# BayesWatch/deep-kernel-transfer

Hardware: AMD Instinct MI355X
Metric: episodes/sec (higher is better)
Workload: dtype f32/f16x2-split

## Files before the change

deep-kernel-transfer_amd/csrc/dkt_mll.h:

```cpp
#pragma once
#include "dkt_common.h"
#include "../../include/dkt_abi.h"

struct MllArgs {
    const float* E;
    const float* Y;
    long y_bstride;
    const float* sv;
    const float* mean;
    const float* noise;
    const float* cls_weight;
    float* logp;
    float* alpha;
    float* L;
    float* W;
    float* dsv;
    float* dmean;
    float* dnoise;
    float* jitter_used;
    int32_t* info;
    float* ws;
    const int32_t* only_failed;
    int b0;
    int B, C, N, LD;
    float jitter0;
    int max_tries;
    unsigned flags;
    int p2_guard;
    float kappa_max = 0.f;
};

constexpr float DKT_HALF_LOG_2PI = 0.91893853320467274178f;

bool dkt_mll_h2_launch(const MllArgs& a, hipStream_t st);
bool dkt_mll_mfma_launch(const MllArgs& a, hipStream_t st);
bool dkt_mll_reg_launch(const MllArgs& a, hipStream_t st);

void dkt_chol_inv_block_launch(const float* A, int lda, long sA, float* L, int ldl, long sL, float* U, int ldu, long sU, int nb,
                               int pivot_base, int32_t* info, int nmat, hipStream_t st);
size_t dkt_mll_big_workspace_bytes(int B, int C, int N);
int dkt_mll_big_launch(const MllArgs& a, void* workspace, size_t ws_bytes, hipStream_t st);
bool dkt_mll_tiled_supports(int N, unsigned flags, int C = 1);
size_t dkt_mll_tiled_workspace_bytes(int B, int C, int N);
size_t dkt_mll_tiled_workspace_bytes_form(int B, int C, int N, bool per_class);
int dkt_mll_tiled_launch(const MllArgs& a, void* workspace, size_t ws_bytes, hipStream_t st);
bool dkt_mll_band_supports(int N, unsigned flags, int C);
bool dkt_mll_band_applies(int B, int C, int N, unsigned flags);
size_t dkt_mll_band_workspace_bytes(int B, int C, int N);
int dkt_mll_band_launch(const MllArgs& a, void* workspace, size_t ws_bytes, hipStream_t st);
void dkt_mll_generic_global_launch(MllArgs a, int b0, int count, float* ws, hipStream_t st);
size_t dkt_mll_generic_global_floats(int count, int N);
```

deep-kernel-transfer_amd/csrc/dkt_mll.hip:

```cpp
#include "dkt_mll.h"
#include <cstdlib>

namespace {

constexpr size_t MLL_LDS_LIMIT = 150 * 1024;

__host__ __device__ inline int mll_ld(int N) { return N | 1; }
inline size_t mll_vec_floats(int N) { return (size_t)3 * (N + 1) + 32; }
inline size_t mll_mat_floats(int N) { return (size_t)(N + 1) * mll_ld(N); }
inline bool mll_fits_lds(int N) { return (mll_vec_floats(N) + mll_mat_floats(N)) * 4 <= MLL_LDS_LIMIT; }

template <bool GLOBAL>
__global__ __launch_bounds__(256) void mll_generic_kernel(MllArgs a) {
    extern __shared__ __attribute__((aligned(16))) float smem[];
    const int tid = threadIdx.x;
    const int tx = tid & 15, ty = tid >> 4;
    const int N = a.N, C = a.C, LD = a.LD, R = N + 1;
    const bool epc = (a.flags & DKT_MLL_E_PER_CLASS) != 0;
    const size_t unit = epc ? (size_t)a.b0 * C + blockIdx.x : (size_t)a.b0 + blockIdx.x;
    const int b = epc ? (int)(unit / (size_t)C) : (int)unit;
    const int c_first = epc ? (int)(unit % (size_t)C) : 0, c_end = epc ? c_first + 1 : C;
    if (a.only_failed) {
        bool need = false;
        for (int c = c_first; c < c_end; ++c) need = need || a.only_failed[(size_t)b * C + c] != 0;
        if (!need) return;
        __syncthreads();
    }
    float* cs = smem;
    float* ldiag = cs + R;
    float* al = ldiag + R;
    float* red = al + R;
    float* Mw = GLOBAL ? (a.ws + (size_t)blockIdx.x * R * LD) : (red + 32);
#define MW(p, j) Mw[(p) * LD + (j)]

    const float* Eb = a.E + unit * N * N;
    const bool want_grad = (a.flags & DKT_MLL_WANT_GRAD) != 0;
    const bool want_chol = (a.flags & DKT_MLL_WANT_CHOL) != 0;
    float* Wb = want_grad ? a.W + unit * N * N : nullptr;

    for (int c = c_first; c < c_end; ++c) {
        const float svc = a.sv[c], mc = a.mean[c], nzc = a.noise[c];
        const float* yc = a.Y + (size_t)b * a.y_bstride + (size_t)c * N;
        int fail_at = 0;
        float jit = 0.f;
        for (int attempt = 0; attempt <= a.max_tries; ++attempt) {
            jit = 0.f;
            if (attempt > 0) {
                jit = a.jitter0;
                for (int i = 1; i < attempt; ++i) jit *= 10.f;
            }
            __syncthreads();
            for (int idx = tid; idx < N * N; idx += 256) {
                const int p = idx / N, j = idx - p * N;
                float v = 0.f;
                if (p >= j) {
                    v = svc * Eb[idx];
                    if (p == j) v += nzc + jit;
                }
                MW(p, j) = v;
            }
            for (int j = tid; j < N; j += 256) MW(N, j) = yc[j] - mc;
            __syncthreads();
            fail_at = 0;
            for (int k = 0; k < N; ++k) {
                const float d = MW(k, k);
                if (!(d > 0.f)) { fail_at = k + 1; break; }
                const float lkk = sqrtf(d);
                const float rinv = 1.0f / lkk;
                for (int p = tid; p < R; p += 256) {
                    if (p != k) {
                        const float v = MW(p, k) * rinv;
                        cs[p] = v;
                        MW(p, k) = v;
                    } else {
                        cs[p] = rinv;
                        ldiag[k] = lkk;
                    }
                }
                __syncthreads();
                for (int p = ty; p < R; p += 16) {
                    const bool low = p <= k;
                    const float cp = cs[p];
                    for (int j = k + 1 + tx; j < N; j += 16) {
                        if (low || p >= j) MW(p, j) -= cp * cs[j];
                    }
                }
                __syncthreads();
            }
            if (fail_at == 0) break;
        }
        __syncthreads();
        const size_t bc = (size_t)b * C + c;
        if (fail_at != 0) {
            const float qnan = __int_as_float(0x7fc00000);
            if (tid == 0) {
                a.logp[bc] = qnan;
                a.jitter_used[bc] = jit;
                a.info[bc] = fail_at;
                if (want_grad) { a.dsv[bc] = qnan; a.dmean[bc] = qnan; a.dnoise[bc] = qnan; }
            }
            for (int i = tid; i < N; i += 256) a.alpha[bc * N + i] = qnan;
            if (want_grad)
                for (int idx = tid; idx < N * N; idx += 256) Wb[idx] = qnan;
            if (want_chol)
                for (int idx = tid; idx < N * N; idx += 256) a.L[bc * N * N + idx] = qnan;
            continue;
        }
        for (int k = tid; k < N; k += 256) MW(k, k) = 1.0f / ldiag[k];
        __syncthreads();
        float qpart = 0.f, lpart = 0.f;
        for (int k = tid; k < N; k += 256) {
            const float w = MW(N, k);
            qpart += w * w;
            lpart += logf(ldiag[k]);
        }
        const float quad = block_sum_256(qpart, red);
        const float logdet_half = block_sum_256(lpart, red);
        float apart = 0.f;
        for (int i = tid; i < N; i += 256) {
            float s = 0.f;
            for (int m = i; m < N; ++m) s += MW(i, m) * MW(N, m);
            al[i] = s;
            a.alpha[bc * N + i] = s;
            apart += s;
        }
        const float asum = block_sum_256(apart, red);
        if (tid == 0) {
            a.logp[bc] = -0.5f * quad - logdet_half - (float)N * DKT_HALF_LOG_2PI;
            a.jitter_used[bc] = jit;
            a.info[bc] = 0;
        }
        if (want_chol) {
            float* Lb = a.L + bc * N * N;
            for (int idx = tid; idx < N * N; idx += 256) {
                const int p = idx / N, j = idx - p * N;
                Lb[idx] = (p > j) ? MW(p, j) : (p == j ? ldiag[p] : 0.f);
            }
        }
        if (want_grad) {
            const float cw = a.cls_weight ? a.cls_weight[c] : 1.0f;
            const float coef = cw * svc;
            float dsv_part = 0.f, tr_part = 0.f;
            for (int i = ty; i < N; i += 16) {
                for (int j = tx; j <= i; j += 16) {
                    float kinv = 0.f;
                    for (int m = i; m < N; ++m) kinv += MW(i, m) * MW(j, m);
                    const float mcv = 0.5f * (al[i] * al[j] - kinv);
                    const float e = Eb[(size_t)i * N + j];
                    if (i == j) { dsv_part += mcv * e; tr_part += mcv; }
                    else dsv_part += 2.0f * mcv * e;
                    const float wv = coef * mcv;
                    if (c == c_first) {
                        Wb[(size_t)i * N + j] = wv;
                        if (i != j) Wb[(size_t)j * N + i] = wv;
                    } else {
                        Wb[(size_t)i * N + j] += wv;
                        if (i != j) Wb[(size_t)j * N + i] += wv;
                    }
                }
            }
            const float dsv = block_sum_256(dsv_part, red);
            const float trm = block_sum_256(tr_part, red);
            if (tid == 0) {
                a.dsv[bc] = dsv;
                a.dmean[bc] = asum;
                a.dnoise[bc] = trm;
            }
        }
    }
#undef MW
}

}

size_t dkt_mll_generic_global_floats(int count, int N) { return (size_t)count * mll_mat_floats(N); }

void dkt_mll_generic_global_launch(MllArgs a, int b0, int count, float* ws, hipStream_t st) {
    a.b0 = b0; a.ws = ws; a.LD = mll_ld(a.N);
    const int units = (a.flags & DKT_MLL_E_PER_CLASS) ? count * a.C : count;
    hipLaunchKernelGGL(mll_generic_kernel<true>, dim3(units), dim3(256), mll_vec_floats(a.N) * sizeof(float), st, a);
}

constexpr float MLL_H2_KAPPA_MAX = 5.0e3f;

static bool mll_kappa_guarded(const MllArgs& a) { return !(a.flags & DKT_MLL_NO_KAPPA_GUARD) && mll_fits_lds(a.N); }

static void mll_kappa_fixup(MllArgs a, hipStream_t st) {
    if (!mll_kappa_guarded(a)) return;
    const int upe = (a.flags & DKT_MLL_E_PER_CLASS) ? a.C : 1;
    const size_t units = (size_t)a.B * upe;
    a.only_failed = a.info;
    a.b0 = 0; a.LD = mll_ld(a.N);
    const size_t lds = (mll_vec_floats(a.N) + mll_mat_floats(a.N)) * sizeof(float);
    if (lds > 48 * 1024 && hipFuncSetAttribute((const void*)mll_generic_kernel<false>, hipFuncAttributeMaxDynamicSharedMemorySize, (int)lds) != hipSuccess) return;
    hipLaunchKernelGGL(mll_generic_kernel<false>, dim3((unsigned)units), dim3(256), lds, st, a);
}

static int g_mll_env_read = 0, g_p2_guard = 1, g_force_f32mfma = 0;
void dkt_mll_reload_env() { g_mll_env_read = 0; }

extern "C" size_t dkt_mll_workspace_bytes(int B, int C, int N) {
    if (B <= 0 || N <= 0 || C <= 0) return 0;
    if (N + 1 <= 128) return 0;
    const size_t big = dkt_mll_big_workspace_bytes(B, C, N);
    const size_t gen = mll_fits_lds(N) ? 0 : (size_t)B * mll_mat_floats(N) * sizeof(float);
    const size_t til = dkt_mll_tiled_supports(N, 0) ? dkt_mll_tiled_workspace_bytes(B, C, N) : 0;
    const size_t bnd = dkt_mll_band_supports(N, 0, C) ? dkt_mll_band_workspace_bytes(B, C, N) : 0;
    size_t mx = big > gen ? big : gen;
    mx = mx > bnd ? mx : bnd;
    return mx > til ? mx : til;
}

extern "C" size_t dkt_mll_workspace_bytes_for(int B, int C, int N, unsigned flags) {
    if (B <= 0 || N <= 0 || C <= 0) return 0;
    const bool pc = (flags & DKT_MLL_E_PER_CLASS) != 0;
    const size_t gen = mll_fits_lds(N) ? 0 : (size_t)(pc ? (B < 128 ? B : 128) * C : B) * mll_mat_floats(N) * sizeof(float);
    if (flags & DKT_MLL_FORCE_GENERIC) return gen;
    if (N + 1 <= 128) return (flags & DKT_MLL_WANT_CHOL) && (N + 1 + 15) / 16 > 2 ? gen : 0;
    if (dkt_mll_band_applies(B, C, N, flags)) return dkt_mll_band_workspace_bytes(B, C, N);
    if (!(flags & DKT_MLL_FORCE_BLOCKED) && dkt_mll_tiled_supports(N, flags, C)) return dkt_mll_tiled_workspace_bytes_form(B, C, N, pc);
    if (pc) return gen;
    const size_t big = dkt_mll_big_workspace_bytes(B, C, N);
    return big > gen ? big : gen;
}

extern "C" int dkt_mll_f32(const float* E, const float* Y, long y_bstride, const float* sv, const float* mean,
                           const float* noise, int B, int C, int N, float jitter0, int max_tries,
                           unsigned flags, const float* cls_weight, float* logp, float* alpha, float* L,
                           float* W, float* dsv, float* dmean, float* dnoise, float* jitter_used,
                           int32_t* info, void* workspace, size_t workspace_bytes, void* stream) {
    if (!E || !Y || !sv || !mean || !noise || !logp || !alpha || !jitter_used || !info) return DKT_ERR_BAD_ARG;
    if (B <= 0 || C <= 0 || N <= 0 || max_tries < 0 || max_tries > 8 || y_bstride < 0) return DKT_ERR_BAD_ARG;
    if ((flags & DKT_MLL_WANT_GRAD) && (!W || !dsv || !dmean || !dnoise)) return DKT_ERR_BAD_ARG;
    if ((flags & DKT_MLL_WANT_CHOL) && !L) return DKT_ERR_BAD_ARG;
    MllArgs a;
    a.E = E; a.Y = Y; a.y_bstride = y_bstride; a.sv = sv; a.mean = mean; a.noise = noise;
    a.cls_weight = cls_weight; a.logp = logp; a.alpha = alpha; a.L = L; a.W = W; a.dsv = dsv;
    a.dmean = dmean; a.dnoise = dnoise; a.jitter_used = jitter_used; a.info = info;
    a.ws = (float*)workspace; a.only_failed = nullptr; a.b0 = 0; a.B = B; a.C = C; a.N = N; a.LD = mll_ld(N);
    a.jitter0 = jitter0; a.max_tries = max_tries; a.flags = flags;
    if (g_mll_env_read == 0) {
        const char* pg = dkt_variant_env("DKT_MLL_P2_GUARD");
        g_p2_guard = pg ? atoi(pg) : 1;
        const char* fm = getenv("DKT_MLL_F32MFMA");
        g_force_f32mfma = (fm && fm[0] == '1') ? 1 : 0;
        g_mll_env_read = 1;
    }
    a.p2_guard = g_p2_guard;
    if (g_force_f32mfma && !(flags & (DKT_MLL_E_PER_CLASS | DKT_MLL_FORCE_GENERIC | DKT_MLL_FORCE_REG | DKT_MLL_FORCE_BLOCKED))) {
        flags |= DKT_MLL_FORCE_F32MFMA;
        a.flags = flags;
    }
    hipStream_t st = (hipStream_t)stream;
    if (flags & DKT_MLL_FORCE_REG) return DKT_ERR_BAD_ARG;
    if (flags & DKT_MLL_E_PER_CLASS) {
        if (flags & (DKT_MLL_WANT_CHOL | DKT_MLL_FORCE_REG | DKT_MLL_FORCE_F32MFMA | DKT_MLL_FORCE_BLOCKED)) return DKT_ERR_BAD_ARG;
        if (!(flags & DKT_MLL_FORCE_GENERIC)) {
            if (N + 1 > 128 && dkt_mll_tiled_supports(N, flags, C)) {
                if (!workspace || workspace_bytes < dkt_mll_tiled_workspace_bytes_form(B, C, N, true)) return DKT_ERR_WORKSPACE;
                return dkt_mll_tiled_launch(a, workspace, workspace_bytes, st);
            }
            if (N + 1 <= 128) {
                a.kappa_max = mll_kappa_guarded(a) ? MLL_H2_KAPPA_MAX : 0.f;
                if (!dkt_mll_h2_launch(a, st)) return DKT_ERR_BAD_ARG;
                mll_kappa_fixup(a, st);
                return hipGetLastError() == hipSuccess ? DKT_OK : DKT_ERR_LAUNCH;
            }
        }
    }
    a.kappa_max = (N + 1 <= 128 && mll_kappa_guarded(a)) ? MLL_H2_KAPPA_MAX : 0.f;
    if (!(flags & (DKT_MLL_FORCE_GENERIC | DKT_MLL_FORCE_REG | DKT_MLL_FORCE_F32MFMA)) && dkt_mll_h2_launch(a, st)) {
        mll_kappa_fixup(a, st);
        return hipGetLastError() == hipSuccess ? DKT_OK : DKT_ERR_LAUNCH;
    }
    if (!(flags & (DKT_MLL_FORCE_GENERIC | DKT_MLL_FORCE_REG)) && dkt_mll_mfma_launch(a, st)) return hipGetLastError() == hipSuccess ? DKT_OK : DKT_ERR_LAUNCH;
    if (dkt_mll_band_applies(B, C, N, flags) && workspace && workspace_bytes >= dkt_mll_band_workspace_bytes(B, C, N))
        return dkt_mll_band_launch(a, workspace, workspace_bytes, st);
    if (!(flags & (DKT_MLL_FORCE_GENERIC | DKT_MLL_FORCE_REG | DKT_MLL_FORCE_BLOCKED)) && dkt_mll_tiled_supports(N, flags, C) && workspace &&
        workspace_bytes >= dkt_mll_tiled_workspace_bytes_form(B, C, N, false))
        return dkt_mll_tiled_launch(a, workspace, workspace_bytes, st);
    if (!(flags & (DKT_MLL_FORCE_GENERIC | DKT_MLL_E_PER_CLASS)) && N + 1 > 128 && workspace && workspace_bytes >= dkt_mll_big_workspace_bytes(B, C, N))
        return dkt_mll_big_launch(a, workspace, workspace_bytes, st);
    const int upe = (flags & DKT_MLL_E_PER_CLASS) ? C : 1;
    if (mll_fits_lds(N)) {
        const size_t lds = (mll_vec_floats(N) + mll_mat_floats(N)) * sizeof(float);
        if (lds > 48 * 1024) {
            if (hipFuncSetAttribute((const void*)mll_generic_kernel<false>,
                                    hipFuncAttributeMaxDynamicSharedMemorySize, (int)lds) != hipSuccess)
                return DKT_ERR_LAUNCH;
        }
        hipLaunchKernelGGL(mll_generic_kernel<false>, dim3((unsigned)B * upe), dim3(256), lds, st, a);
    } else {
        const size_t per_ep = (size_t)upe * mll_mat_floats(N) * sizeof(float);
        const size_t fit = workspace ? workspace_bytes / per_ep : 0;
        if (fit < 1) return DKT_ERR_WORKSPACE;
        const int cnt = fit < (size_t)B ? (int)fit : B;
        for (int b0 = 0; b0 < B; b0 += cnt) dkt_mll_generic_global_launch(a, b0, (B - b0 < cnt) ? B - b0 : cnt, (float*)workspace, st);
    }
    return hipGetLastError() == hipSuccess ? DKT_OK : DKT_ERR_LAUNCH;
}
```

deep-kernel-transfer_amd/csrc/dkt_mll_h2.hip:

```cpp
#include "dkt_h2_tiles.h"
#include <cstdlib>

namespace {

using namespace dkt_mfma;

#ifndef DKT_H2E_P2H
#define DKT_H2E_P2H 1
#endif
#ifndef DKT_H2_SWEEP_PRIO
#define DKT_H2_SWEEP_PRIO 1
#endif
#define DKT_SWEEP_PRIO(p) do { if (DKT_H2_SWEEP_PRIO) __builtin_amdgcn_s_setprio(p); } while (0)

constexpr int ntt(int nt) { return nt * (nt + 1) / 2; }
__host__ __device__ constexpr int tidx(int i, int j) { return j * (j + 1) / 2 + i; }

constexpr int H2_MAX_WPG = 5;

#ifdef DKT_MFMA_CLOCKS
#define DKT_CLK(i) do { __builtin_amdgcn_sched_barrier(0); clk[i] = __builtin_amdgcn_s_memtime(); __builtin_amdgcn_sched_barrier(0); } while (0)
#else
#define DKT_CLK(i) do { } while (0)
#endif
// ... 398 lines not shown
            float asum = 0.f, aa = 0.f;
            {
                const brsrc ar = mk_rsrc(a.alpha + bc * N, (unsigned)(N * 4));
                const float asc = ldexpf(aug_unscale, -msc);
                float* ysf = reinterpret_cast<float*>(myys);
#pragma unroll
                for (int i = 0; i < NT; ++i) {
                    const f32x4 m = (i < NT - 1) ? T.t[i][NT - 1] : myst[(NT - 1) * 64 + lane];
                    const float v = -(qn == 0 ? m[0] : qn == 1 ? m[1] : qn == 2 ? m[2] : m[3]) * asc;
                    const bool ok = arow && ((i < NT - 1) || (c16 < pN));
                    bstore1(ar, (fail_at != 0) ? qnan : v, ok ? (16 * i + c16) * 4 : OOB, 0);
                    if (GRAD && arow) ysf[16 * i + c16] = ok ? v : 0.f;
                    asum += ok ? v : 0.f;
                    aa += ok ? v * v : 0.f;
                }
            }
            float trk = 0.f;
            DKT_CLK(4);
            if constexpr (GRAD) {
                float mx = 0.f;
#pragma unroll
                for (int i = 0; i < NT - 1; ++i) {
#pragma unroll
                    for (int q = 0; q < 4; ++q) T.t[i][NT - 1][q] = (g4 + q == pN) ? 0.f : T.t[i][NT - 1][q];
                }
#pragma unroll
                for (int j = 1; j < NT; ++j) {
#pragma unroll
                    for (int i = 0; i < j; ++i) {
                        const f32x4 v = T.t[i][j];
                        mx = fmaxf(mx, fmaxf(fmaxf(fabsf(v[0]), fabsf(v[1])), fmaxf(fabsf(v[2]), fabsf(v[3]))));
                    }
                }
#pragma unroll
                for (int j = 0; j < NT; ++j) {
                    const f32x4 v = myst[j * 64 + lane];
#pragma unroll
                    for (int q = 0; q < 4; ++q) mx = fmaxf(mx, (j == NT - 1 && g4 + q == pN) ? 0.f : fabsf(v[q]));
                }
                mx = wave_reduce_dpp<true>(mx);
                mx = __int_as_float(__builtin_amdgcn_readfirstlane(__float_as_int(mx)));
                float s3_inv;
                const float s3 = scale_for(mx, s3_inv);
#pragma unroll
                for (int j = 0; j < NT; ++j) {
                    f32x4 v = myst[j * 64 + lane];
                    if (j == NT - 1) {
#pragma unroll
                        for (int q = 0; q < 4; ++q) v[q] = (g4 + q == pN) ? 0.f : v[q];
                    }
                    myst[j * 64 + lane] = split_h2(v, s3);
                }
#pragma unroll
                for (int j = 1; j < NT; ++j) {
#pragma unroll
                    for (int i = 0; i < j; ++i) T.t[i][j] = split_h2(T.t[i][j], s3);
                }
#pragma unroll
                for (int j = 0; j < NT; ++j) {
                    __builtin_amdgcn_sched_barrier(0);
#pragma unroll
                    for (int i = 0; i <= j; i += 2) {
                        const bool pair = i + 1 <= j;
                        f32x4 accA = {0.f, 0.f, 0.f, 0.f}, accB = {0.f, 0.f, 0.f, 0.f};
#pragma unroll
                        for (int k = j; k < NT; ++k) {
                            const f32x4 Bm = (k == j) ? myst[k * 64 + lane] : T.t[j][k];
                            const f32x4 A0 = (k == i) ? myst[k * 64 + lane] : T.t[i][k];
                            if (pair) {
                                const f32x4 A1 = (k == i + 1) ? myst[k * 64 + lane] : T.t[i + 1][k];
                                xtyh2(A0, Bm, accA, A1, Bm, accB);
                            } else {
                                accA = xtyh(A0, Bm, accA);
                            }
                        }
                        auto put = [&](const f32x4 acc, const int ii) {
                            if (ii < j) {
                                T.t[ii][j] = acc;
                            } else {
                                myst[j * 64 + lane] = acc;
#pragma unroll
                                for (int q = 0; q < 4; ++q) {
                                    const bool ok = (g4 + q == c16) && ((j < NT - 1) || (c16 < pN));
                                    trk += ok ? acc[q] : 0.f;
                                }
                            }
                        };
                        put(accA, i);
                        if (pair) put(accB, i + 1);
                    }
                }
                trk *= s3_inv * s3_inv * ldexpf(1.0f, -2 * msc);
                const float cw = a.cls_weight ? a.cls_weight[c] : 1.0f;
                coefK = (fail_at == 0) ? -0.5f * cw * a.sv[c] * s3_inv * s3_inv * ldexpf(1.0f, -2 * msc) : qnan;
                coefA = 0.5f * cw * a.sv[c];
            }
            DKT_CLK(5);
            lsum = wave_reduce_dpp<false>(lsum) + (float)(2 * msc * N);
            asum = wave_reduce_dpp<false>(asum);
            aa = wave_reduce_dpp<false>(aa);
            trk = wave_reduce_dpp<false>(trk);
            if (lane == 0) {
                const bool ok = fail_at == 0;
                a.logp[bc] = ok ? (-0.5f * quad - 0.34657359027997264f * lsum - (float)N * DKT_HALF_LOG_2PI) : qnan;
                a.jitter_used[bc] = jit;
                a.info[bc] = (ok && kappa_high) ? -1 : fail_at;
                if constexpr (GRAD) {
                    const float nz_eff = a.noise[c] + jit;
                    const float trpp = trk - aa;
                    a.dmean[bc] = ok ? asum : qnan;
                    a.dnoise[bc] = ok ? -0.5f * trpp : qnan;
                    a.dsv[bc] = ok ? 0.5f * ((quad - (float)N) + nz_eff * trpp) / a.sv[c] : qnan;
                }
            }
        }
        DKT_CLK(6);
        if constexpr (GRAD) {
            __syncthreads();
            tq = tid;
            DKT_OPAQUE_V(tq);
            c16 = tq & 15; g4 = (tq >> 2) & 12; lane = tq & 63;
            DKT_OPAQUE_S(N);
            const int pNs = N - 16 * (NT - 1);
            const brsrc Wr = mk_rsrc(a.W + (size_t)unit * N * N, (unsigned)(N * N * 4));
            const float* alf = reinterpret_cast<const float*>(myys);
            auto scaled_tile = [&](const f32x4 p, const int i, const int j) {
                const f32x4 ar = myys[4 * i + (g4 >> 2)];
                const float ac = alf[16 * j + c16] * coefA;
                f32x4 v;
#pragma unroll
                for (int q = 0; q < 4; ++q) v[q] = fmaf(ar[q], ac, p[q] * coefK);
                return v;
            };
            auto store_tile = [&](f32x4 v, const int i, const int j) {
                const bool col_ok = (j < NT - 1) || (c16 < pNs);
                const int vo_m = col_ok ? ((16 * j + c16) * N + 16 * i + g4) * 4 : OOB;
                int vo_d[4], vo_t[4];
#pragma unroll
                for (int q = 0; q < 4; ++q) {
                    const bool row_ok = (i < NT - 1) || (g4 + q < pNs);
                    const bool keep = row_ok && col_ok && (i < j || g4 + q <= c16);
                    vo_d[q] = keep ? ((16 * i + g4 + q) * N + 16 * j + c16) * 4 : OOB;
                    vo_t[q] = (keep && g4 + q < c16) ? ((16 * j + c16) * N + 16 * i + g4 + q) * 4 : OOB;
                }
                if (round > 0) {
                    if (i < j) {
                        v += bload4(Wr, vo_m, 0);
                    } else {
#pragma unroll
                        for (int q = 0; q < 4; ++q) v[q] += __uint_as_float(__builtin_amdgcn_raw_buffer_load_b32(Wr, vo_d[q], 0, 0));
                    }
                }
#pragma unroll
                for (int q = 0; q < 4; ++q) bstore1(Wr, v[q], vo_d[q], 0);
                if (i < j) bstore4(Wr, v, vo_m, 0);
                else {
#pragma unroll
                    for (int q = 0; q < 4; ++q) bstore1(Wr, v[q], vo_t[q], 0);
                }
            };
            if constexpr (WPG5) {
                constexpr int KMAX = (NTT + 4) / 5;
#pragma unroll
                for (int g = 0; g < 5; ++g) {
                    if (ep_ok) {
#pragma unroll
                        for (int j = 0; j < NT; ++j) {
#pragma unroll
                            for (int i = 0; i <= j; ++i) {
                                const int n = tidx(i, j);
                                if (n % 5 != g) continue;
                                f32x4 v = {0.f, 0.f, 0.f, 0.f};
                                if (active) v = scaled_tile((i < j) ? T.t[i][j] : myst[j * 64 + lane], i, j);
                                stage[(w * KMAX + n / 5) * 64 + lane] = v;
                            }
                        }
                    }
                    __syncthreads();
                    if (ep_ok) {
                        for (int k = w; 5 * k + g < NTT; k += 5) {
                            f32x4 v = stage[k * 64 + lane];
#pragma unroll
                            for (int ww = 1; ww < 5; ++ww) v += stage[(ww * KMAX + k) * 64 + lane];
                            const int n = 5 * k + g;
                            int j = 0;
                            while ((j + 1) * (j + 2) / 2 <= n) ++j;
                            store_tile(v, n - j * (j + 1) / 2, j);
                        }
                    }
                    if (g < 4 || round + 1 < nrounds) __syncthreads();
                }
            } else {
                for (int t = 0; t < wpg; ++t) {
                    if (t == w && active) {
#pragma unroll
                        for (int j = 0; j < NT; ++j) {
#pragma unroll
                            for (int i = 0; i <= j; ++i) {
                                f32x4 v = scaled_tile((i < j) ? T.t[i][j] : myst[j * 64 + lane], i, j);
                                f32x4* p = &stage[tidx(i, j) * 64 + lane];
                                if (t > 0) v += *p;
                                *p = v;
                            }
                        }
                    }
                    __syncthreads();
                }
                if (ep_ok) {
                    for (int n = w; n < NTT; n += wpg) {
                        int j = 0;
                        while ((j + 1) * (j + 2) / 2 <= n) ++j;
                        store_tile(stage[n * 64 + lane], n - j * (j + 1) / 2, j);
                    }
                }
                if (round + 1 < nrounds) __syncthreads();
            }
        } else {
            if (round + 1 < nrounds) __syncthreads();
        }
    }
    DKT_CLK(7);
#ifdef DKT_MFMA_CLOCKS
    DKT_CLK(8);
    if ((tid & 63) == 0 && a.ws) {
        unsigned long long* o = reinterpret_cast<unsigned long long*>(a.ws) + ((size_t)blockIdx.x * (H2_MAX_WPG * EPW) + wall) * 48;
        for (int i = 0; i < 32; ++i) o[i] = clk[i];
    }
#endif
}

template <int NT> constexpr int h2e_wlds() { return ntt(NT) < 19 ? ntt(NT) : 19; }

template <int NT>
__global__ __attribute__((amdgpu_flat_work_group_size(64, 64), amdgpu_waves_per_eu(2, 2)))
void mll_h2e_kernel(MllArgs a) {
    constexpr int WLDS = h2e_wlds<NT>();
    constexpr int WREG = ntt(NT) - WLDS;
    __shared__ f32x4 wl[WLDS * 64];
    __shared__ f32x4 yst[NT * 4];

    const bool epc = (a.flags & DKT_MLL_E_PER_CLASS) != 0;
    const bool want_grad = (a.flags & DKT_MLL_WANT_GRAD) != 0;
    const int C = a.C;
    const int b = epc ? (int)(blockIdx.x / (unsigned)C) : (int)blockIdx.x;
    const int c_first = epc ? (int)(blockIdx.x % (unsigned)C) : 0, c_end = epc ? c_first + 1 : C;
    const size_t mat = epc ? (size_t)b * C + c_first : (size_t)b;
    const float qnan = __int_as_float(0x7fc00000);
    int tq = threadIdx.x;
    DKT_OPAQUE_V(tq);
    int c16 = tq & 15, g4 = (tq >> 2) & 12, lane = tq & 63, N = a.N;
    DKT_OPAQUE_S(N);

    f32x4 wr[WREG > 0 ? WREG : 1];
#pragma unroll
    for (int n = 0; n < WREG; ++n) wr[n] = (f32x4){0.f, 0.f, 0.f, 0.f};
#pragma unroll
    for (int n = 0; n < WLDS; ++n) wl[n * 64 + lane] = (f32x4){0.f, 0.f, 0.f, 0.f};
#ifdef DKT_MFMA_CLOCKS
    unsigned long long ph[8] = {}, tprev = __builtin_amdgcn_s_memtime();
#define DKT_PH(i) do { __builtin_amdgcn_sched_barrier(0); const unsigned long long tn = __builtin_amdgcn_s_memtime(); ph[i] += tn - tprev; tprev = tn; __builtin_amdgcn_sched_barrier(0); } while (0)
#else
#define DKT_PH(i) do { } while (0)
#endif
    int e_acc = -1000;
    float sigma = 0.f;
    bool poison = false;

    int attempt = 0;
    for (int c = c_first; c < c_end;) {
        tq = threadIdx.x;
        DKT_OPAQUE_V(tq);
        c16 = tq & 15; g4 = (tq >> 2) & 12; lane = tq & 63; N = a.N;
        DKT_OPAQUE_S(N);
        const int pN = N - 16 * (NT - 1);
        Lane ln;
        ln.lane = lane; ln.g = g4 >> 2; ln.c = c16;
        ln.g0 = ln.g == 0; ln.g1 = ln.g == 1; ln.g2 = ln.g == 2;
        const float svc = a.sv[c], mc = a.mean[c], nzc = a.noise[c];
        const size_t bc = (size_t)b * C + c;
        float r2 = 0.f;
        {
            const brsrc yr = mk_rsrc(a.Y + (size_t)b * a.y_bstride + (size_t)c * N, (unsigned)(N * 4));
            float* ysf = reinterpret_cast<float*>(yst);
            {
                const float yv = __uint_as_float(__builtin_amdgcn_raw_buffer_load_b32(yr, lane * 4, 0, 0));
                if (lane < 16 * NT) ysf[lane] = yv;
                r2 = (lane < N) ? (yv - mc) * (yv - mc) : 0.f;
            }
            if (NT > 4 && lane + 64 < 16 * NT) {
                const float yv = __uint_as_float(__builtin_amdgcn_raw_buffer_load_b32(yr, (lane + 64) * 4, 0, 0));
                ysf[lane + 64] = yv;
                r2 += (lane + 64 < N) ? (yv - mc) * (yv - mc) : 0.f;
            }
        }
        r2 = wave_reduce_dpp<false>(r2);
        h4 negIh;
#pragma unroll
        for (int q = 0; q < 4; ++q) negIh[q] = (g4 + q == c16) ? (_Float16)-1.0f : (_Float16)0.0f;
        FormCtxT<true> f;
        f.es = nullptr; f.ys = yst;
        f.pN = pN; f.c16 = c16; f.g4 = g4; f.lane = lane; f.mc = mc;
        Tiles<NT> T;
        int fail_at = 0;
        bool kappa_high = false;
        float jit = 0.f, lsum = 0.f, quad = 0.f, aug_unscale = 1.f;
        int msc = 0;
        const brsrc Er = mk_rsrc(a.E + mat * N * N, (unsigned)(N * N * 4));
        {
            if (attempt > 0) {
                jit = a.jitter0;
                for (int i = 1; i < attempt; ++i) jit *= 10.f;
            }
            load_all_e<NT>(T, Er, N, pN, c16, g4);
            float emax = 0.f, etr = 0.f;
#pragma unroll
            for (int j = 0; j < NT; ++j) {
#pragma unroll
                for (int q = 0; q < 4; ++q) {
                    emax = fmaxf(emax, (g4 + q == c16) ? T.t[j][j][q] : 0.f);
                    etr += (g4 + q == c16) ? T.t[j][j][q] : 0.f;
                }
            }
            emax = wave_reduce_dpp<true>(emax);
            kappa_high = a.kappa_max > 0.f && !(1.0f + svc * wave_reduce_dpp<false>(etr) / nzc <= a.kappa_max);
            int ex;
            (void)frexpf(fmaf(svc, emax, nzc + jit), &ex);
            msc = max(0, (ex + 1) >> 1);
            const float ikap = ldexpf(1.0f, -2 * msc);
            const float lam = fmaxf((nzc + jit) * ikap, 9.094947017729282e-13f);
            int exm;
            (void)frexpf(1.0f / lam, &exm);
            const int emu = (exm + 1) >> 1;
            int exr;
            (void)frexpf(r2 * ikap * ldexpf(1.0f, 2 * emu), &exr);
            const int er = (r2 > 0.f) ? ((exr + 1) >> 1) : 0;
            f.nsv = -svc * ikap * TWO30;
            f.dg = -(nzc + jit) * ikap * TWO30;
            f.rsc = ldexpf(TWO30, -msc - er);
            aug_unscale = ldexpf(1.0f, er);
            form_row0<NT, 0>(T, f);
            DKT_PH(0);
            P1Ctx pc;
            pc.myst = nullptr; pc.negIh = negIh;
            pc.lane = lane; pc.c16 = c16; pc.pN = pN;
            pc.fail_at = 0; pc.lsum = 0.f; pc.quad = 0.f;
#ifdef DKT_MFMA_CLOCKS
            unsigned long long clkdummy[32];
            pc.clk = clkdummy;
#endif
            {
                float dv, x[16];
                sweep_begin30(T.t[0][0], x, dv);
                sweep_interleaved<NT, -1, 0, NT == 1>(T, f, x, dv, ln, pN);
                phase1_step<NT, 0>(T, f, pc, x, dv, ln);
            }
            fail_at = pc.fail_at; lsum = pc.lsum; quad = pc.quad * aug_unscale * aug_unscale;
        }
        DKT_PH(1);
        if (fail_at != 0 && attempt < a.max_tries) {
            ++attempt;
            continue;
        }
        tq = threadIdx.x;
        DKT_OPAQUE_V(tq);
        c16 = tq & 15; g4 = (tq >> 2) & 12; lane = tq & 63;
#if DKT_H2E_P2H
        const float cw = a.cls_weight ? a.cls_weight[c] : 1.0f;
        const float wmag = 0.5f * fabsf(cw) * svc;
        const float gsc = (wmag > 0.f) ? __builtin_sqrtf(wmag) * ldexpf(1.0f, -msc) : ldexpf(1.0f, -msc);
        const bool arow = (ln.g == (pN >> 2));
        const int qn = pN & 3;
        const float asc = ldexpf(aug_unscale, -msc);
        float asum = 0.f, aa = 0.f;
        const brsrc ar = mk_rsrc(a.alpha + bc * N, (unsigned)(N * 4));
        float* ysf = reinterpret_cast<float*>(yst);
        auto emit_alpha = [&](const float v, const int i) {
            const bool ok = arow && ((i < NT - 1) || (c16 < pN));
            bstore1(ar, (fail_at != 0) ? qnan : v, ok ? (16 * i + c16) * 4 : OOB, 0);
            if (arow) ysf[16 * i + c16] = ok ? v : 0.f;
            asum += ok ? v : 0.f;
            aa += ok ? v * v : 0.f;
        };
        {
            const f32x4 m = T.t[NT - 1][NT - 1];
            emit_alpha(-(qn == 0 ? m[0] : qn == 1 ? m[1] : qn == 2 ? m[2] : m[3]) * asc, NT - 1);
        }
        float mx = 0.f, mxt0 = 0.f;
#pragma unroll
        for (int j = 0; j < NT; ++j) {
            const f32x4 v = T.t[j][j];
            mx = fmaxf(mx, fmaxf(fmaxf(fabsf(v[0]), fabsf(v[1])), fmaxf(fabsf(v[2]), fabsf(v[3]))));
            if (j == 0) mxt0 = mx;
        }
        mx = wave_reduce_dpp<true>(mx);
        const float mx0 = __int_as_float(__builtin_amdgcn_readfirstlane(__float_as_int(mx)));
        if (a.p2_guard < 0) mx = wave_reduce_dpp<true>(mxt0);
        mx = __int_as_float(__builtin_amdgcn_readfirstlane(__float_as_int(mx * gsc)));
        const bool sane = (fail_at == 0) && (mx > 0.f) && (mx < 3.0e38f) && (mx0 < 3.0e38f);
        const float unitX = sane ? ldexpf(1.0f, 15 - ((int)((__float_as_uint(mx0) >> 23) & 0xffu) - 126)) : 1.0f;
        int e2 = (int)((__float_as_uint(mx) >> 23) & 0xffu) - 126 + max(a.p2_guard, 0);
        if (sigma != 0.f) e2 = max(e2, e_acc);
        e2 = sane ? min(max(e2, -100), 100) : 0;
        float unit2 = ldexpf(1.0f, 15 - e2);
        bool ovf = false;
        auto zero_aug_row = [&](f32x4 v) {
#pragma unroll
            for (int q = 0; q < 4; ++q) v[q] = (g4 + q == pN) ? 0.f : v[q];
            return v;
        };
        auto scale_planes = [&](const f32x4 raw, const _Float16 f) {
            Sp sp = as_sp(raw);
            sp.h = sp.h * f;
            sp.m = sp.m * f;
            return __builtin_bit_cast(f32x4, sp);
        };
#pragma unroll
        for (int j = 1; j < NT; ++j) {
            __builtin_amdgcn_sched_barrier(0);
            const f32x4 nV = neg_transpose_h2(split_h2(T.t[j][j], unitX), negIh);
            T.t[j - 1][j - 1] = split_h2(T.t[j - 1][j - 1], gsc * unit2);
            float mrow = 0.f;
#pragma unroll
            for (int i = 0; i < j; i += 2) {
                if (i + 1 < j) {
                    f32x4 QA = xtyh0(T.t[i][j], T.t[i][i]);
                    f32x4 QB = {0.f, 0.f, 0.f, 0.f};
#pragma unroll
                    for (int k = i + 1; k < j; ++k) xtyh2(T.t[k][j], T.t[i][k], QA, T.t[k][j], T.t[i + 1][k], QB);
                    f32x4 RA = {0.f, 0.f, 0.f, 0.f}, RB = {0.f, 0.f, 0.f, 0.f};
                    xtyh2(nV, split_h2(QA, 1.1920928955078125e-07f), RA, nV, split_h2(QB, 1.1920928955078125e-07f), RB);
                    T.t[i][j] = RA;
                    T.t[i + 1][j] = RB;
                    mrow = fmaxf(mrow, fmaxf(fmaxf(fmaxf(fabsf(RA[0]), fabsf(RA[1])), fmaxf(fabsf(RA[2]), fabsf(RA[3]))),
                                             fmaxf(fmaxf(fabsf(RB[0]), fabsf(RB[1])), fmaxf(fabsf(RB[2]), fabsf(RB[3])))));
                } else {
                    f32x4 Q = xtyh0(T.t[i][j], T.t[i][i]);
#pragma unroll
                    for (int k = i + 1; k < j; ++k) Q = xtyh(T.t[k][j], T.t[i][k], Q);
                    const f32x4 RA = xtyh0(nV, split_h2(Q, 1.1920928955078125e-07f));
                    T.t[i][j] = RA;
                    mrow = fmaxf(mrow, fmaxf(fmaxf(fabsf(RA[0]), fabsf(RA[1])), fmaxf(fabsf(RA[2]), fabsf(RA[3]))));
                }
            }
            {
                const f32x4 v = T.t[j][j];
                const float md = fmaxf(fmaxf(fabsf(v[0]), fabsf(v[1])), fmaxf(fabsf(v[2]), fabsf(v[3])));
                mrow = fmaxf(mrow * (256.0f / unitX), md * gsc * unit2);
            }
            mrow = wave_reduce_dpp<true>(mrow);
            const float ymax = __int_as_float(__builtin_amdgcn_readfirstlane(__float_as_int(mrow)));
            float fac = 256.0f / unitX;
            ovf = ovf || !(ymax < 3.0e38f);
            if (sane && ymax >= 32768.0f && ymax < 3.0e38f) {
                const int dgrow = (int)((__float_as_uint(ymax) >> 23) & 0xffu) - 126 - 15;
                const _Float16 fh = (_Float16)ldexpf(1.0f, -dgrow);
#pragma unroll
                for (int k = 0; k < j; ++k) {
#pragma unroll
                    for (int i = 0; i <= k; ++i) T.t[i][k] = scale_planes(T.t[i][k], fh);
                }
                e2 += dgrow;
                unit2 = ldexpf(unit2, -dgrow);
                fac = ldexpf(fac, -dgrow);
            }
            if (j == NT - 1) {
                const float aun = fac / (gsc * unit2) * asc;
#pragma unroll
                for (int i = 0; i < NT - 1; ++i) {
                    const f32x4 m = T.t[i][NT - 1];
                    emit_alpha(-(qn == 0 ? m[0] : qn == 1 ? m[1] : qn == 2 ? m[2] : m[3]) * aun, i);
                }
            }
#pragma unroll
            for (int i = 0; i < j; ++i) T.t[i][j] = split_h2((j == NT - 1) ? zero_aug_row(T.t[i][j]) : T.t[i][j], fac);
        }
        T.t[NT - 1][NT - 1] = split_h2(zero_aug_row(T.t[NT - 1][NT - 1]), gsc * unit2);
        if (ovf && fail_at == 0) fail_at = N + 1;
        DKT_PH(2);
        DKT_PH(3);
        tq = threadIdx.x;
        DKT_OPAQUE_V(tq);
        c16 = tq & 15; g4 = (tq >> 2) & 12; lane = tq & 63;
        const bool live = want_grad && (fail_at == 0) && (wmag > 0.f) && sane;
        poison = poison || (fail_at != 0);
        float trk = 0.f;
        if (live) {
            const int e_c = e2;
            const float sg = (cw > 0.f) ? -1.0f : 1.0f;
            const bool first = sigma == 0.f;
            const bool flip = !first && sg != sigma;
            const bool grow = !first && e_c > e_acc;
            if (flip || grow) {
                const float fac = (flip ? -1.0f : 1.0f) * (grow ? ldexpf(1.0f, -2 * (e_c - e_acc)) : 1.0f);
#pragma unroll
                for (int n = 0; n < WREG; ++n) wr[n] *= fac;
#pragma unroll
                for (int n = 0; n < WLDS; ++n) wl[n * 64 + lane] = wl[n * 64 + lane] * fac;
            }
            e_acc = e_c;
            sigma = sg;
            const float unit = ldexpf(1.0f, 15 - e_acc);
#else
        f32x4 negI2;
#pragma unroll
        for (int q = 0; q < 4; ++q) negI2[q] = (g4 + q == c16) ? -TWOM15 : 0.0f;
#pragma unroll
        for (int j = 1; j < NT; ++j) {
            __builtin_amdgcn_sched_barrier(0);
            const f32x4 nV = xty0(T.t[j][j], negI2);
#pragma unroll
            for (int k = 0; k < j; ++k) T.t[k][j] = join_h2(T.t[k][j]);
#pragma unroll
            for (int i = 0; i < j; i += 2) {
                if (i + 1 < j) {
                    f32x4 QA = xty0(T.t[i][j], T.t[i][i]);
                    f32x4 QB = {0.f, 0.f, 0.f, 0.f};
#pragma unroll
                    for (int k = i + 1; k < j; ++k) xty2(T.t[k][j], T.t[i][k], QA, T.t[k][j], T.t[i + 1][k], QB);
                    f32x4 RA = {0.f, 0.f, 0.f, 0.f}, RB = {0.f, 0.f, 0.f, 0.f};
                    xty2(nV, QA, RA, nV, QB, RB);
                    T.t[i][j] = RA;
                    T.t[i + 1][j] = RB;
                } else {
                    f32x4 Q = xty0(T.t[i][j], T.t[i][i]);
#pragma unroll
                    for (int k = i + 1; k < j; ++k) Q = xty(T.t[k][j], T.t[i][k], Q);
                    T.t[i][j] = xty0(nV, Q);
                }
            }
        }
        DKT_PH(2);
        const bool arow = (ln.g == (pN >> 2));
        const int qn = pN & 3;
        float asum = 0.f, aa = 0.f;
        {
            const brsrc ar = mk_rsrc(a.alpha + bc * N, (unsigned)(N * 4));
            const float asc = ldexpf(aug_unscale, -msc);
            float* ysf = reinterpret_cast<float*>(yst);
#pragma unroll
            for (int i = 0; i < NT; ++i) {
                const f32x4 m = T.t[i][NT - 1];
                const float v = -(qn == 0 ? m[0] : qn == 1 ? m[1] : qn == 2 ? m[2] : m[3]) * asc;
                const bool ok = arow && ((i < NT - 1) || (c16 < pN));
                bstore1(ar, (fail_at != 0) ? qnan : v, ok ? (16 * i + c16) * 4 : OOB, 0);
                if (arow) ysf[16 * i + c16] = ok ? v : 0.f;
                asum += ok ? v : 0.f;
                aa += ok ? v * v : 0.f;
            }
        }
        DKT_PH(3);
        tq = threadIdx.x;
        DKT_OPAQUE_V(tq);
        c16 = tq & 15; g4 = (tq >> 2) & 12; lane = tq & 63;
        const float cw = a.cls_weight ? a.cls_weight[c] : 1.0f;
        const float wmag = 0.5f * fabsf(cw) * svc;
        const float gsc = __builtin_sqrtf(wmag) * ldexpf(1.0f, -msc);
        float mx = 0.f;
#pragma unroll
        for (int i = 0; i < NT; ++i) {
#pragma unroll
            for (int q = 0; q < 4; ++q) T.t[i][NT - 1][q] = (g4 + q == pN) ? 0.f : T.t[i][NT - 1][q];
        }
#pragma unroll
        for (int j = 0; j < NT; ++j) {
#pragma unroll
            for (int i = 0; i <= j; ++i) {
                const f32x4 v = T.t[i][j];
                mx = fmaxf(mx, fmaxf(fmaxf(fabsf(v[0]), fabsf(v[1])), fmaxf(fabsf(v[2]), fabsf(v[3]))));
            }
        }
        mx = wave_reduce_dpp<true>(mx) * gsc;
        mx = __int_as_float(__builtin_amdgcn_readfirstlane(__float_as_int(mx)));
        const bool live = want_grad && (fail_at == 0) && (wmag > 0.f) && (mx > 0.f) && (mx < 3.0e38f);
        poison = poison || (fail_at != 0);
        float trk = 0.f;
        if (live) {
            const int e_c = (int)((__float_as_uint(mx) >> 23) & 0xffu) - 126;
            const float sg = (cw > 0.f) ? -1.0f : 1.0f;
            const bool first = sigma == 0.f;
            const bool flip = !first && sg != sigma;
            const bool grow = !first && e_c > e_acc;
            if (flip || grow) {
                const float fac = (flip ? -1.0f : 1.0f) * (grow ? ldexpf(1.0f, -2 * (e_c - e_acc)) : 1.0f);
#pragma unroll
                for (int n = 0; n < WREG; ++n) wr[n] *= fac;
#pragma unroll
                for (int n = 0; n < WLDS; ++n) wl[n * 64 + lane] = wl[n * 64 + lane] * fac;
            }
            e_acc = first ? e_c : max(e_acc, e_c);
            sigma = sg;
            const float unit = ldexpf(1.0f, 15 - e_acc);
            const float qsc = gsc * unit;
#pragma unroll
            for (int j = 0; j < NT; ++j) {
#pragma unroll
                for (int i = 0; i <= j; ++i) T.t[i][j] = split_h2(T.t[i][j], qsc);
            }
#endif
            const float* alf = reinterpret_cast<const float*>(yst);
            const float ca = -wmag * unit * unit;
#pragma unroll
            for (int j = 0; j < NT; ++j) {
                __builtin_amdgcn_sched_barrier(0);
                const float acol = alf[16 * j + c16] * ca;
#pragma unroll
                for (int i = 0; i <= j; i += 2) {
                    const bool pair = i + 1 <= j;
                    auto cin = [&](const int ii) {
                        const f32x4 ar = yst[4 * ii + (g4 >> 2)];
                        const int n = tidx(ii, j);
                        f32x4 cacc = {0.f, 0.f, 0.f, 0.f};
                        if (ii < j) {
                            if (n < WLDS) cacc = wl[n * 64 + lane];
                            else cacc = wr[n - WLDS < 0 ? 0 : n - WLDS];
                        }
#pragma unroll
                        for (int q = 0; q < 4; ++q) cacc[q] = fmaf(ar[q], acol, cacc[q]);
                        return cacc;
                    };
                    f32x4 accA = cin(i), accB = pair ? cin(i + 1) : (f32x4){0.f, 0.f, 0.f, 0.f};
#pragma unroll
                    for (int k = j; k < NT; ++k) {
                        const f32x4 Bm = T.t[j][k];
                        if (pair) xtyh2(T.t[i][k], Bm, accA, T.t[i + 1][k], Bm, accB);
                        else accA = xtyh(T.t[i][k], Bm, accA);
                    }
                    auto put = [&](const f32x4 acc, const int ii) {
                        const int n = tidx(ii, j);
                        if (ii < j) {
                            if (n < WLDS) wl[n * 64 + lane] = acc;
                            else wr[n - WLDS < 0 ? 0 : n - WLDS] = acc;
                        } else {
#pragma unroll
                            for (int q = 0; q < 4; ++q) {
                                const bool ok = (g4 + q == c16) && ((j < NT - 1) || (c16 < pN));
                                trk += ok ? acc[q] : 0.f;
                            }
                            if (n < WLDS) wl[n * 64 + lane] = wl[n * 64 + lane] + acc;
                            else wr[n - WLDS < 0 ? 0 : n - WLDS] += acc;
                        }
                    };
                    put(accA, i);
                    if (pair) put(accB, i + 1);
                }
            }
            trk *= 1.0f / (wmag * unit * unit);
        }
        DKT_PH(4);
        lsum = wave_reduce_dpp<false>(lsum) + (float)(2 * msc * N);
        asum = wave_reduce_dpp<false>(asum);
        aa = wave_reduce_dpp<false>(aa);
        trk = wave_reduce_dpp<false>(trk);
        if (want_grad && !live && fail_at == 0) {
            float fro = 0.f;
#pragma unroll
            for (int j = 0; j < NT; ++j) {
#pragma unroll
                for (int i = 0; i <= j; ++i) {
#if DKT_H2E_P2H
                    const f32x4 u = join_h2(T.t[i][j]);
#else
                    const f32x4 u = T.t[i][j];
#endif
#pragma unroll
                    for (int q = 0; q < 4; ++q) fro += (j < NT - 1 || g4 + q < pN) ? u[q] * u[q] : 0.f;
                }
            }
#if DKT_H2E_P2H
            trk = wave_reduce_dpp<false>(fro) * ldexpf(1.0f, -2 * msc) / (gsc * gsc * unit2 * unit2) - aa;
#else
            trk = wave_reduce_dpp<false>(fro) * ldexpf(1.0f, -2 * msc) - aa;
#endif
        }
        if (lane == 0) {
            const bool ok = fail_at == 0;
            a.logp[bc] = ok ? (-0.5f * quad - 0.34657359027997264f * lsum - (float)N * DKT_HALF_LOG_2PI) : qnan;
            a.jitter_used[bc] = jit;
            a.info[bc] = (ok && kappa_high) ? -1 : fail_at;
            if (want_grad) {
                const float nz_eff = nzc + jit;
                a.dmean[bc] = ok ? asum : qnan;
                a.dnoise[bc] = ok ? -0.5f * trk : qnan;
                a.dsv[bc] = ok ? 0.5f * ((quad - (float)N) + nz_eff * trk) / svc : qnan;
            }
        }
        DKT_PH(5);
        attempt = 0;
        ++c;
    }
    if (want_grad) {
        tq = threadIdx.x;
        DKT_OPAQUE_V(tq);
        c16 = tq & 15; g4 = (tq >> 2) & 12; lane = tq & 63; N = a.N;
        DKT_OPAQUE_S(N);
        const int pN = N - 16 * (NT - 1);
        const float fin = poison ? qnan : ((sigma == 0.f) ? 0.f : sigma * ldexpf(1.0f, -2 * (15 - e_acc)));
        const brsrc Wr = mk_rsrc(a.W + mat * N * N, (unsigned)(N * N * 4));
#pragma unroll
        for (int j = 0; j < NT; ++j) {
            const bool col_ok = (j < NT - 1) || (c16 < pN);
#pragma unroll
            for (int i = 0; i <= j; ++i) {
                const int n = tidx(i, j);
                f32x4 v;
                if (n < WLDS) v = wl[n * 64 + lane];
                else v = wr[n - WLDS < 0 ? 0 : n - WLDS];
#pragma unroll
                for (int q = 0; q < 4; ++q) v[q] = poison ? qnan : v[q] * fin;
                if (i < j) {
                    bstore4(Wr, v, col_ok ? ((16 * j + c16) * N + 16 * i + g4) * 4 : OOB, 0);
#pragma unroll
                    for (int q = 0; q < 4; ++q) {
                        const bool row_ok = (i < NT - 1) || (g4 + q < pN);
                        bstore1(Wr, v[q], (row_ok && col_ok) ? ((16 * i + g4 + q) * N + 16 * j + c16) * 4 : OOB, 0);
                    }
                } else {
#pragma unroll
                    for (int q = 0; q < 4; ++q) {
                        const bool row_ok = (i < NT - 1) || (g4 + q < pN);
                        const bool keep = row_ok && col_ok && g4 + q <= c16;
                        bstore1(Wr, v[q], keep ? ((16 * i + g4 + q) * N + 16 * j + c16) * 4 : OOB, 0);
                        bstore1(Wr, v[q], (keep && g4 + q < c16) ? ((16 * j + c16) * N + 16 * i + g4 + q) * 4 : OOB, 0);
                    }
                }
            }
        }
    }
#ifdef DKT_MFMA_CLOCKS
    DKT_PH(6);
    if (lane == 0 && a.ws) {
        unsigned long long* o = reinterpret_cast<unsigned long long*>(a.ws) + (size_t)blockIdx.x * 8;
        for (int i = 0; i < 7; ++i) o[i] = ph[i];
        o[7] = __builtin_amdgcn_s_getreg((4 << 0) | (0 << 6) | (31 << 11));
    }
#endif
}

int g_h2e_minb = -1;
int h2e_min_batch() {
    if (g_h2e_minb < 0) { const char* e = getenv("DKT_MLL_H2E_MINB"); g_h2e_minb = e ? atoi(e) : 1024; }
    return g_h2e_minb;
}

template <int NT>
void launch_h2(const MllArgs& a, hipStream_t st) {
    const bool g = (a.flags & DKT_MLL_WANT_GRAD) != 0;
    if constexpr (NT <= 7) {
        if (a.flags & DKT_MLL_E_PER_CLASS) {
            hipLaunchKernelGGL((mll_h2e_kernel<NT>), dim3(a.B * a.C), dim3(64), 0, st, a);
            return;
        }
        if (g && a.B >= h2e_min_batch()) {
            hipLaunchKernelGGL((mll_h2e_kernel<NT>), dim3(a.B), dim3(64), 0, st, a);
            return;
        }
    }
    const bool epc = (a.flags & DKT_MLL_E_PER_CLASS) != 0;
    const int rounds = (a.C + H2_MAX_WPG - 1) / H2_MAX_WPG;
    const int wpg = epc ? 1 : (a.C + rounds - 1) / rounds;
    constexpr int EPW = h2_epw<NT>();
    const dim3 grid(((epc ? a.B * a.C : a.B) + EPW - 1) / EPW), block(64 * wpg * EPW);
    if (g && wpg == 5) hipLaunchKernelGGL((mll_h2_kernel<NT, true, true>), grid, block, 0, st, a, wpg);
    else if (g) hipLaunchKernelGGL((mll_h2_kernel<NT, true, false>), grid, block, 0, st, a, wpg);
    else hipLaunchKernelGGL((mll_h2_kernel<NT, false, false>), grid, block, 0, st, a, wpg);
}

}

void dkt_mll_h2_reload_env() { g_h2e_minb = -1; }

bool dkt_mll_h2_launch(const MllArgs& a, hipStream_t st) {
    if (a.flags & DKT_MLL_WANT_CHOL) return false;
    const int nt = (a.N + 1 + 15) / 16;
    switch (nt) {
        case 1: launch_h2<1>(a, st); return true;
        case 2: launch_h2<2>(a, st); return true;
        case 3: launch_h2<3>(a, st); return true;
        case 4: launch_h2<4>(a, st); return true;
        case 5: launch_h2<5>(a, st); return true;
        case 6: launch_h2<6>(a, st); return true;
        case 7: launch_h2<7>(a, st); return true;
        case 8: launch_h2<8>(a, st); return true;
        default: return false;
    }
}
```

Baseline: 2.078 million.

## Replace per-tile dynamic rescale with a static bound and fallback on violation

In the h2e kernel's gradient path, the per-column-tile wave reduction and dynamic f16 rescale (growth) step is replaced by a static a priori scale exponent derived from gsc and emu, with a single running-max reduction at the end. If the bound is violated, the unit is flagged with info=-1 and its gradient is skipped. The kappa fixup generic kernel is then extended to recompute only negatively flagged units even when the kappa guard is disabled. This removes several cross-lane reductions and branches per tile, at the cost of occasional fallback recomputation on the slow generic kernel and added code complexity. The old dynamic growth path is only compiled in under DKT_TWINS and used only when an env variable is set.

```diff
diff --git a/deep-kernel-transfer_amd/csrc/dkt_mll.h b/deep-kernel-transfer_amd/csrc/dkt_mll.h
--- a/deep-kernel-transfer_amd/csrc/dkt_mll.h
+++ b/deep-kernel-transfer_amd/csrc/dkt_mll.h
@@ -27,12 +27,15 @@
     int max_tries;
     unsigned flags;
     int p2_guard;
+    int p2_grow = 0;
+    int only_negative = 0;
     float kappa_max = 0.f;
 };
 
 constexpr float DKT_HALF_LOG_2PI = 0.91893853320467274178f;
 
 bool dkt_mll_h2_launch(const MllArgs& a, hipStream_t st);
+bool dkt_mll_h2e_serves(const MllArgs& a);
 bool dkt_mll_mfma_launch(const MllArgs& a, hipStream_t st);
 bool dkt_mll_reg_launch(const MllArgs& a, hipStream_t st);
 
diff --git a/deep-kernel-transfer_amd/csrc/dkt_mll.hip b/deep-kernel-transfer_amd/csrc/dkt_mll.hip
--- a/deep-kernel-transfer_amd/csrc/dkt_mll.hip
+++ b/deep-kernel-transfer_amd/csrc/dkt_mll.hip
@@ -22,7 +22,10 @@
     const int c_first = epc ? (int)(unit % (size_t)C) : 0, c_end = epc ? c_first + 1 : C;
     if (a.only_failed) {
         bool need = false;
-        for (int c = c_first; c < c_end; ++c) need = need || a.only_failed[(size_t)b * C + c] != 0;
+        for (int c = c_first; c < c_end; ++c) {
+            const int32_t f = a.only_failed[(size_t)b * C + c];
+            need = need || (a.only_negative ? f < 0 : f != 0);
+        }
         if (!need) return;
         __syncthreads();
     }
@@ -186,7 +189,10 @@
 static bool mll_kappa_guarded(const MllArgs& a) { return !(a.flags & DKT_MLL_NO_KAPPA_GUARD) && mll_fits_lds(a.N); }
 
 static void mll_kappa_fixup(MllArgs a, hipStream_t st) {
-    if (!mll_kappa_guarded(a)) return;
+    if (!mll_kappa_guarded(a)) {
+        if (!mll_fits_lds(a.N) || !dkt_mll_h2e_serves(a)) return;
+        a.only_negative = 1;
+    }
     const int upe = (a.flags & DKT_MLL_E_PER_CLASS) ? a.C : 1;
     const size_t units = (size_t)a.B * upe;
     a.only_failed = a.info;
@@ -196,7 +202,7 @@
     hipLaunchKernelGGL(mll_generic_kernel<false>, dim3((unsigned)units), dim3(256), lds, st, a);
 }
 
-static int g_mll_env_read = 0, g_p2_guard = 1, g_force_f32mfma = 0;
+static int g_mll_env_read = 0, g_p2_guard = 1, g_p2_grow = 0, g_force_f32mfma = 0;
 void dkt_mll_reload_env() { g_mll_env_read = 0; }
 
 extern "C" size_t dkt_mll_workspace_bytes(int B, int C, int N) {
@@ -242,11 +248,12 @@
     if (g_mll_env_read == 0) {
         const char* pg = dkt_variant_env("DKT_MLL_P2_GUARD");
         g_p2_guard = pg ? atoi(pg) : 1;
+        g_p2_grow = pg ? 1 : 0;
         const char* fm = getenv("DKT_MLL_F32MFMA");
         g_force_f32mfma = (fm && fm[0] == '1') ? 1 : 0;
         g_mll_env_read = 1;
     }
-    a.p2_guard = g_p2_guard;
+    a.p2_guard = g_p2_guard; a.p2_grow = g_p2_grow;
     if (g_force_f32mfma && !(flags & (DKT_MLL_E_PER_CLASS | DKT_MLL_FORCE_GENERIC | DKT_MLL_FORCE_REG | DKT_MLL_FORCE_BLOCKED))) {
         flags |= DKT_MLL_FORCE_F32MFMA;
         a.flags = flags;
diff --git a/deep-kernel-transfer_amd/csrc/dkt_mll_h2.hip b/deep-kernel-transfer_amd/csrc/dkt_mll_h2.hip
--- a/deep-kernel-transfer_amd/csrc/dkt_mll_h2.hip
+++ b/deep-kernel-transfer_amd/csrc/dkt_mll_h2.hip
@@ -724,9 +724,9 @@
         f.pN = pN; f.c16 = c16; f.g4 = g4; f.lane = lane; f.mc = mc;
         Tiles<NT> T;
         int fail_at = 0;
-        bool kappa_high = false;
+        bool kappa_high = false, bviol = false;
         float jit = 0.f, lsum = 0.f, quad = 0.f, aug_unscale = 1.f;
-        int msc = 0;
+        int msc = 0, emu = 0;
         const brsrc Er = mk_rsrc(a.E + mat * N * N, (unsigned)(N * N * 4));
         {
             if (attempt > 0) {
@@ -752,7 +752,7 @@
             const float lam = fmaxf((nzc + jit) * ikap, 9.094947017729282e-13f);
             int exm;
             (void)frexpf(1.0f / lam, &exm);
-            const int emu = (exm + 1) >> 1;
+            emu = (exm + 1) >> 1;
             int exr;
             (void)frexpf(r2 * ikap * ldexpf(1.0f, 2 * emu), &exr);
             const int er = (r2 > 0.f) ? ((exr + 1) >> 1) : 0;
@@ -787,6 +787,11 @@
         DKT_OPAQUE_V(tq);
         c16 = tq & 15; g4 = (tq >> 2) & 12; lane = tq & 63;
 #if DKT_H2E_P2H
+#ifdef DKT_TWINS
+        const bool p2grow = a.p2_grow != 0;
+#else
+        constexpr bool p2grow = false;
+#endif
         const float cw = a.cls_weight ? a.cls_weight[c] : 1.0f;
         const float wmag = 0.5f * fabsf(cw) * svc;
         const float gsc = (wmag > 0.f) ? __builtin_sqrtf(wmag) * ldexpf(1.0f, -msc) : ldexpf(1.0f, -msc);
@@ -816,15 +821,17 @@
         }
         mx = wave_reduce_dpp<true>(mx);
         const float mx0 = __int_as_float(__builtin_amdgcn_readfirstlane(__float_as_int(mx)));
-        if (a.p2_guard < 0) mx = wave_reduce_dpp<true>(mxt0);
+        if (p2grow && a.p2_guard < 0) mx = wave_reduce_dpp<true>(mxt0);
         mx = __int_as_float(__builtin_amdgcn_readfirstlane(__float_as_int(mx * gsc)));
         const bool sane = (fail_at == 0) && (mx > 0.f) && (mx < 3.0e38f) && (mx0 < 3.0e38f);
         const float unitX = sane ? ldexpf(1.0f, 15 - ((int)((__float_as_uint(mx0) >> 23) & 0xffu) - 126)) : 1.0f;
         int e2 = (int)((__float_as_uint(mx) >> 23) & 0xffu) - 126 + max(a.p2_guard, 0);
+        if (!p2grow) e2 = (int)((__float_as_uint(gsc * ldexpf(1.0f, emu)) >> 23) & 0xffu) - 126 + 1;
         if (sigma != 0.f) e2 = max(e2, e_acc);
         e2 = sane ? min(max(e2, -100), 100) : 0;
         float unit2 = ldexpf(1.0f, 15 - e2);
         bool ovf = false;
+        float mrun = 0.f;
         auto zero_aug_row = [&](f32x4 v) {
 #pragma unroll
             for (int q = 0; q < 4; ++q) v[q] = (g4 + q == pN) ? 0.f : v[q];
@@ -864,16 +871,18 @@
                     mrow = fmaxf(mrow, fmaxf(fmaxf(fabsf(RA[0]), fabsf(RA[1])), fmaxf(fabsf(RA[2]), fabsf(RA[3]))));
                 }
             }
-            {
+            float fac = 256.0f / unitX;
+            if (!p2grow) mrun = fmaxf(mrun, mrow);
+            float ymax = 0.f;
+            if (p2grow) {
                 const f32x4 v = T.t[j][j];
                 const float md = fmaxf(fmaxf(fabsf(v[0]), fabsf(v[1])), fmaxf(fabsf(v[2]), fabsf(v[3])));
                 mrow = fmaxf(mrow * (256.0f / unitX), md * gsc * unit2);
-            }
-            mrow = wave_reduce_dpp<true>(mrow);
-            const float ymax = __int_as_float(__builtin_amdgcn_readfirstlane(__float_as_int(mrow)));
-            float fac = 256.0f / unitX;
-            ovf = ovf || !(ymax < 3.0e38f);
-            if (sane && ymax >= 32768.0f && ymax < 3.0e38f) {
+                mrow = wave_reduce_dpp<true>(mrow);
+                ymax = __int_as_float(__builtin_amdgcn_readfirstlane(__float_as_int(mrow)));
+                ovf = ovf || !(ymax < 3.0e38f);
+            }
+            if (p2grow && sane && ymax >= 32768.0f && ymax < 3.0e38f) {
                 const int dgrow = (int)((__float_as_uint(ymax) >> 23) & 0xffu) - 126 - 15;
                 const _Float16 fh = (_Float16)ldexpf(1.0f, -dgrow);
 #pragma unroll
@@ -897,13 +906,19 @@
             for (int i = 0; i < j; ++i) T.t[i][j] = split_h2((j == NT - 1) ? zero_aug_row(T.t[i][j]) : T.t[i][j], fac);
         }
         T.t[NT - 1][NT - 1] = split_h2(zero_aug_row(T.t[NT - 1][NT - 1]), gsc * unit2);
+        if (!p2grow) {
+            mrun = wave_reduce_dpp<true>(mrun);
+            const float ymax = fmaxf(__int_as_float(__builtin_amdgcn_readfirstlane(__float_as_int(mrun))) * (256.0f / unitX), mx * unit2);
+            ovf = !(ymax < 3.0e38f);
+            bviol = sane && !ovf && ymax >= 32768.0f;
+        }
         if (ovf && fail_at == 0) fail_at = N + 1;
         DKT_PH(2);
         DKT_PH(3);
         tq = threadIdx.x;
         DKT_OPAQUE_V(tq);
         c16 = tq & 15; g4 = (tq >> 2) & 12; lane = tq & 63;
-        const bool live = want_grad && (fail_at == 0) && (wmag > 0.f) && sane;
+        const bool live = want_grad && (fail_at == 0) && (wmag > 0.f) && sane && !bviol;
         poison = poison || (fail_at != 0);
         float trk = 0.f;
         if (live) {
@@ -1098,7 +1113,7 @@
             const bool ok = fail_at == 0;
             a.logp[bc] = ok ? (-0.5f * quad - 0.34657359027997264f * lsum - (float)N * DKT_HALF_LOG_2PI) : qnan;
             a.jitter_used[bc] = jit;
-            a.info[bc] = (ok && kappa_high) ? -1 : fail_at;
+            a.info[bc] = (ok && (kappa_high || bviol)) ? -1 : fail_at;
             if (want_grad) {
                 const float nz_eff = nzc + jit;
                 a.dmean[bc] = ok ? asum : qnan;
@@ -1187,6 +1202,11 @@
     else hipLaunchKernelGGL((mll_h2_kernel<NT, false, false>), grid, block, 0, st, a, wpg);
 }
 
+}
+
+bool dkt_mll_h2e_serves(const MllArgs& a) {
+    if ((a.flags & DKT_MLL_WANT_CHOL) || (a.N + 1 + 15) / 16 > 7) return false;
+    return (a.flags & DKT_MLL_E_PER_CLASS) || ((a.flags & DKT_MLL_WANT_GRAD) && a.B >= h2e_min_batch());
 }
 
 void dkt_mll_h2_reload_env() { g_h2e_minb = -1; }
```

New measurement: 2.076 million. No clear change (-0.1%).
